# raahii/dcvgan

Hardware: AMD Instinct MI355X
Metric: videos/sec per G+D step, 16x64x64 RGB+depth (higher is better)
Workload: dtype f32

## Files before the change

### dcvgan_amd/csrc/conv_mfma.hip

```cpp
#include "dcv_common.h"

#include <algorithm>
#include <cstdlib>
#include <map>
#include <mutex>
#include <string>
#include <type_traits>
#include <vector>

namespace dcv {

thread_local char g_err[512] = {0};
std::atomic<uint64_t> g_launches{0};
thread_local char g_last_kernel[160] = {0};
#define DCV_NOTE_KERNEL(...) snprintf(g_last_kernel, sizeof(g_last_kernel), __VA_ARGS__)

typedef float f32x16 __attribute__((ext_vector_type(16)));
typedef __bf16 bf16x8 __attribute__((ext_vector_type(8)));

std::atomic<int> g_precision{0};
struct BnView {
    const float* bx; const float* gamma; const float* beta; const float* mean; const float* invstd;
    int64_t bx_sn;
    int32_t bx_sc, bx_sh, cbn, act;
// ... 1409 lines not shown
    uint32_t plane, gb;
    xcd_plane_map(blockIdx.x, gpp, gridDim.x, plane, gb);
    const uint32_t n = plane / (uint32_t)a.OD, od = plane - n * (uint32_t)a.OD;
    int32_t kb4[KS];
    uint32_t padmask = 0, b0mask = 0, b2mask = 0, r0mask = 0, r1mask = 0, r2mask = 0;
#pragma unroll
    for (int m = 0; m < KS; ++m) {
        const int k = 2 * m + lhi;
        const bool live = k < K;
        const int kk = live ? k : 0;
        const int rc = kk / 9, t = kk - rc * 9, ra = t / 3, b = t - ra * 3;
        kb4[m] = rc * a.s_stepA + 4 * (ra * a.x_sh + b);
        padmask |= live ? 0u : 1u << m;
        b0mask |= (live && b == 0) ? 1u << m : 0u;
        b2mask |= (live && b == 2) ? 1u << m : 0u;
        r0mask |= (live && ra == 0) ? 1u << m : 0u;
        r1mask |= (live && ra == 1) ? 1u << m : 0u;
        r2mask |= (live && ra == 2) ? 1u << m : 0u;
    }
    const __amdgpu_buffer_rsrc_t xrs = __builtin_amdgcn_make_buffer_rsrc(
        const_cast<float*>(a.x + (int64_t)n * a.x_sn + (int64_t)((int)od * a.td.mul + a.td.base + a.td.delta[0]) * a.x_sd), 0, 0x80000000u, 0x00020000);
    const __amdgpu_buffer_rsrc_t yrs = __builtin_amdgcn_make_buffer_rsrc(a.y + a.y_off + (int64_t)n * a.y_sn + (int64_t)od * a.y_sd, 0, 0x80000000u, 0x00020000);
    const __amdgpu_buffer_rsrc_t bxrs = __builtin_amdgcn_make_buffer_rsrc(const_cast<float*>(h.bx + (int64_t)n * h.bx_sn), 0, 0x80000000u, 0x00020000);
    const __amdgpu_buffer_rsrc_t bdrs = __builtin_amdgcn_make_buffer_rsrc((MODE == 2 ? h.bdx : a.y) + (MODE == 2 ? (int64_t)n * h.bdx_sn : 0), 0, 0x80000000u, 0x00020000);
    const int ysh = (int)a.y_sh, ysw = (int)a.y_sw;
    const uint32_t ysc4 = (uint32_t)a.y_sc * 4u, bxsc4 = (uint32_t)h.bx_sc * 4u, bdsc4 = (uint32_t)h.bdx_sc * 4u;
    const float slope = h.slope;

    auto load_b = [&](int oh, int x0, float (&bv)[KS]) {
        const int ih0 = oh + a.p_ihmin;
        const int col = x0 + l31;
        uint32_t bad = padmask | (col == 0 ? b0mask : 0u) | (col == a.tw.size - 1 ? b2mask : 0u);
        if ((unsigned)ih0 >= (unsigned)a.th.size) bad |= r0mask;
        if ((unsigned)(ih0 + 1) >= (unsigned)a.th.size) bad |= r1mask;
        if ((unsigned)(ih0 + 2) >= (unsigned)a.th.size) bad |= r2mask;
        const int base4 = 4 * (ih0 * a.x_sh + col - 1);
#pragma unroll
        for (int m = 0; m < KS; ++m) {
            const uint32_t vo = ((bad >> m) & 1u) ? 0x80000000u : (uint32_t)(base4 + kb4[m]);
            bv[m] = __builtin_bit_cast(float, __builtin_amdgcn_raw_buffer_load_b32(xrs, vo, 0, 0));
        }
    };

    const int ntile = groups * 2;
    __syncthreads();
    const int ohw = (int)gb * groups * 4 + wave * groups;
    const int mt_end = MODE == 2 ? MB : MT;
#pragma unroll 1
    for (int mt = 0; mt < mt_end; ++mt) {
        const bool bn = mt < MB;
        float af[KS];
#pragma unroll
        for (int m = 0; m < KS; ++m) af[m] = wl[2 * m + lhi][mt * 32 + l31];
        float s1[16], s2[16];
#pragma unroll
        for (int r = 0; r < 16; ++r) { s1[r] = 0.f; s2[r] = 0.f; }
        float bcur[KS], bnxt[KS];
        load_b(ohw, 0, bcur);
#pragma unroll 1
        for (int tt = 0; tt < ntile; ++tt) {
            const int oh = ohw + (tt >> 1), x0 = (tt & 1) * 32;
            float xt[16];
            if (bn) {
                const uint32_t xv = (uint32_t)(4 * (oh * h.bx_sh + (x0 + l31) * h.bx_sw)) + (uint32_t)(4 * lhi) * bxsc4;
#pragma unroll
                for (int r = 0; r < 16; ++r)
                    xt[r] = __builtin_bit_cast(float, __builtin_amdgcn_raw_buffer_load_b32(bxrs, xv, (uint32_t)(mt * 32 + (r & 3) + 8 * (r >> 2)) * bxsc4, 0));
            }
            if (tt + 1 < ntile) load_b(ohw + ((tt + 1) >> 1), ((tt + 1) & 1) * 32, bnxt);
            f32x16 acc;
#pragma unroll
            for (int r = 0; r < 16; ++r) acc[r] = 0.f;
#pragma unroll
            for (int m = 0; m < KS; ++m) acc = __builtin_amdgcn_mfma_f32_32x32x2f32(af[m], bcur[m], acc, 0, 0, 0);
            if (bn) {
                const uint32_t dv = (uint32_t)(4 * (oh * h.bdx_sh + (x0 + l31) * h.bdx_sw)) + (uint32_t)(4 * lhi) * bdsc4;
#pragma unroll
                for (int r = 0; r < 16; ++r) {
                    const int ch = mt * 32 + (r & 3) + 8 * (r >> 2) + 4 * lhi;
                    const f32x4 k4 = c4[ch];
                    const float z = xt[r] * k4[0] + k4[1];
                    const float dz = acc[r] * (z > 0.f ? 1.f : slope);
                    const float xm = xt[r] - k4[2];
                    if (MODE == 1) {
                        s1[r] += dz;
                        s2[r] += dz * xm;
                    } else {
                        const f32x2 k2 = c2[ch];
                        const float o = k4[0] * dz + k2[0] + k2[1] * xm;
                        __builtin_amdgcn_raw_buffer_store_b32(__builtin_bit_cast(int, o), bdrs, dv, (uint32_t)(mt * 32 + (r & 3) + 8 * (r >> 2)) * bdsc4, 2);
                    }
                }
            } else {
                const uint32_t yv = (uint32_t)(4 * (oh * ysh + (x0 + l31) * ysw)) + (uint32_t)(4 * lhi) * ysc4;
#pragma unroll
                for (int r = 0; r < 16; ++r) {
                    const float v = acc[r];
                    __builtin_amdgcn_raw_buffer_store_b32(__builtin_bit_cast(int, v), yrs, yv, (uint32_t)(mt * 32 + (r & 3) + 8 * (r >> 2)) * ysc4, 2);
                }
            }
#pragma unroll
            for (int m = 0; m < KS; ++m) bcur[m] = bnxt[m];
        }
        if (MODE == 1 && bn) {
#pragma unroll
            for (int r = 0; r < 16; ++r) {
                const float t1 = half_wave_sum(s1[r]), t2 = half_wave_sum(s2[r]);
                if (l31 == 31) {
                    const int ch = mt * 32 + (r & 3) + 8 * (r >> 2) + 4 * lhi;
                    red[wave][ch][0] = t1;
                    red[wave][ch][1] = t2;
                }
            }
        }
    }
    if (MODE == 1) {
        __syncthreads();
        if (tid < 2 * cbn) {
            const int ch = tid >> 1, w = tid & 1;
            h.partial[((int64_t)blockIdx.x * cbn + ch) * 2 + w] = ((red[0][ch][w] + red[1][ch][w]) + red[2][ch][w]) + red[3][ch][w];
        }
    }
}

__global__ __launch_bounds__(256) void head_bn_finalize_kernel(const float* __restrict__ partial, int nwg, int cbn, double count, const float* __restrict__ gamma,
                                                               const float* __restrict__ invstd, float* __restrict__ dgamma, float* __restrict__ dbeta, float* __restrict__ cst) {
    __shared__ double red[2][256];
    const int c = blockIdx.x, tid = threadIdx.x;
    double a0 = 0.0, a1 = 0.0;
    for (int w = tid; w < nwg; w += 256) {
        a0 += (double)partial[((int64_t)w * cbn + c) * 2];
        a1 += (double)partial[((int64_t)w * cbn + c) * 2 + 1];
    }
    red[0][tid] = a0; red[1][tid] = a1;
    __syncthreads();
    for (int st = 128; st > 0; st >>= 1) {
        if (tid < st) { red[0][tid] += red[0][tid + st]; red[1][tid] += red[1][tid + st]; }
        __syncthreads();
    }
    if (tid == 0) {
        const double is = (double)invstd[c], sc = (double)gamma[c] * is;
        const double S1 = red[0][0], S2 = red[1][0];
        dbeta[c] = (float)S1;
        dgamma[c] = (float)(S2 * is);
        cst[2 * c] = (float)(-sc * S1 / count);
        cst[2 * c + 1] = (float)(-sc * is * is * S2 / count);
    }
}

struct QuadArgs {
    const float* s;
    float* y;
    const float* w;
    int32_t N, RC, OC, SD, SH, OD, pad0, pad1;
    int64_t s_sn, s_sc, s_sd, s_sh;
    int64_t y_sn, y_sc, y_sd, y_sh;
    int64_t w_o, w_r;
    int32_t act, accumulate;
    float slope, pad2;
};

template <int NOC, int ND>
__global__ __launch_bounds__(256) void thin_quad_kernel(const QuadArgs a) {
    __shared__ float red[3][8 * NOC][64];
    const int tid = threadIdx.x, lane = tid & 63;
    const int wave = __builtin_amdgcn_readfirstlane(tid >> 6);
    const int col = lane & 31, hw = lane >> 5;
    const uint32_t qb = (uint32_t)a.SH >> 2;
    const uint32_t plane = blockIdx.x / qb;
    const int r0 = (int)(blockIdx.x - plane * qb) * 4 + 2 * hw;
    const uint32_t n = plane / (uint32_t)a.OD, od = plane - n * (uint32_t)a.OD;
    int roff[4];
#pragma unroll
    for (int i = 0; i < 4; ++i) {
        const int rr = r0 - 1 + i;
        roff[i] = (unsigned)rr < (unsigned)a.SH ? rr * (int)a.s_sh + col : -1;
    }
    float acc[2][2][2][NOC];
#pragma unroll
    for (int q = 0; q < 2; ++q)
#pragma unroll
        for (int h = 0; h < 2; ++h)
#pragma unroll
            for (int b = 0; b < 2; ++b)
#pragma unroll
                for (int c = 0; c < NOC; ++c) acc[q][h][b][c] = 0.f;
    const float* __restrict__ sn = a.s + (int64_t)n * a.s_sn;
#pragma unroll(ND == 1 ? 4 : 1)
    for (int rc = wave; rc < a.RC; rc += 4) {
        float ctr[ND][4];
#pragma unroll
        for (int kd = 0; kd < ND; ++kd) {
            const int sd = (int)od - kd;
            const bool in = (unsigned)sd < (unsigned)a.SD;
            const float* __restrict__ pl = sn + (int64_t)rc * a.s_sc + (int64_t)(in ? sd : 0) * a.s_sd;
#pragma unroll
            for (int i = 0; i < 4; ++i) ctr[kd][i] = (in && roff[i] >= 0) ? pl[roff[i]] : 0.f;
        }
#pragma unroll
        for (int kd = 0; kd < ND; ++kd) {
            float g[4][3];
#pragma unroll
            for (int i = 0; i < 4; ++i) {
                const float v = ctr[kd][i];
                g[i][1] = v;
                float l = __builtin_bit_cast(float, __builtin_amdgcn_update_dpp(0, __builtin_bit_cast(int, v), 0x138, 0xf, 0xf, true));
                float r = __builtin_bit_cast(float, __builtin_amdgcn_update_dpp(0, __builtin_bit_cast(int, v), 0x130, 0xf, 0xf, true));
                g[i][0] = col == 0 ? 0.f : l;
                g[i][2] = col == 31 ? 0.f : r;
            }
#pragma unroll
            for (int c = 0; c < NOC; ++c) {
                if (c >= a.OC) continue;
                typedef float f32x4 __attribute__((ext_vector_type(4)));
                const f32x4* __restrict__ wq = reinterpret_cast<const f32x4*>(a.w + (int64_t)c * a.w_o + (int64_t)rc * a.w_r + kd * 16);
                const f32x4 w0 = wq[0], w1 = wq[1], w2 = wq[2], w3 = wq[3];
#pragma unroll
                for (int q = 0; q < 2; ++q) {
                    const float (&top)[3] = g[q], (&mid)[3] = g[q + 1], (&bot)[3] = g[q + 2];
                    acc[q][0][0][c] += mid[1] * w1[1] + mid[0] * w1[3] + top[1] * w3[1] + top[0] * w3[3];
                    acc[q][0][1][c] += mid[2] * w1[0] + mid[1] * w1[2] + top[2] * w3[0] + top[1] * w3[2];
                    acc[q][1][0][c] += bot[1] * w0[1] + bot[0] * w0[3] + mid[1] * w2[1] + mid[0] * w2[3];
                    acc[q][1][1][c] += bot[2] * w0[0] + bot[1] * w0[2] + mid[2] * w2[0] + mid[1] * w2[2];
                }
            }
        }
    }
    if (wave > 0) {
#pragma unroll
        for (int q = 0; q < 2; ++q)
#pragma unroll
            for (int h = 0; h < 2; ++h)
#pragma unroll
                for (int b = 0; b < 2; ++b)
#pragma unroll
                    for (int c = 0; c < NOC; ++c) red[wave - 1][((q * 2 + h) * 2 + b) * NOC + c][lane] = acc[q][h][b][c];
    }
    __syncthreads();
    if (wave != 0) return;
    const int OC = a.OC, act = a.act, accumulate = a.accumulate;
    const float slope = a.slope;
    float* __restrict__ yb = a.y + (int64_t)n * a.y_sn + (int64_t)od * a.y_sd + 2 * col;
#pragma unroll
    for (int q = 0; q < 2; ++q)
#pragma unroll
        for (int h = 0; h < 2; ++h)
#pragma unroll
            for (int c = 0; c < NOC; ++c) {
                if (c >= OC) continue;
                float v[2];
#pragma unroll
                for (int b = 0; b < 2; ++b) {
                    const int e = ((q * 2 + h) * 2 + b) * NOC + c;
                    v[b] = acc[q][h][b][c] + ((red[0][e][lane] + red[1][e][lane]) + red[2][e][lane]);
                }
                float* dst = yb + (int64_t)(2 * (r0 + q) + h) * a.y_sh + (int64_t)c * a.y_sc;
                if (accumulate) { v[0] += dst[0]; v[1] += dst[1]; }
                dst[0] = apply_act(v[0], act, slope);
                dst[1] = apply_act(v[1], act, slope);
            }
}

template <int T>
static bool launch_thin_struct(const GatherArgs& a, int OC, int RC, int rc_per_split, dim3 grid, hipStream_t s) {
    switch (OC) {
        case 1: hipLaunchKernelGGL((thin_struct_kernel<T, 1>), grid, dim3(256), 0, s, a, RC, rc_per_split); return true;
        case 2: hipLaunchKernelGGL((thin_struct_kernel<T, 2>), grid, dim3(256), 0, s, a, RC, rc_per_split); return true;
        case 3: hipLaunchKernelGGL((thin_struct_kernel<T, 3>), grid, dim3(256), 0, s, a, RC, rc_per_split); return true;
        case 4: hipLaunchKernelGGL((thin_struct_kernel<T, 4>), grid, dim3(256), 0, s, a, RC, rc_per_split); return true;
    }
    return false;
}

struct PackArgs {
    const KEntry* ktab[4];
    float* wp[4];
    int32_t K16[4];
    int32_t fmt[4];
};
__global__ void pack_weights_kernel(const float* __restrict__ w, const PackArgs pa, int OC, int OCp, int64_t ws_o) {
    const int c = blockIdx.y;
    const int64_t i = (int64_t)blockIdx.x * blockDim.x + threadIdx.x;
    if (i >= (int64_t)pa.K16[c] * OCp) return;
    const int k = (int)(i / OCp), oc = (int)(i % OCp);
    const KEntry e = pa.ktab[c][k];
    float v = 0.f;
    if (oc < OC && !(e.tapsel >> 31)) v = w[(int64_t)oc * ws_o + e.w_off];
    if (pa.fmt[c] == 2) {
        if (X6_PHASE(k >> 4)) v = -v;
        __bf16* o = reinterpret_cast<__bf16*>(pa.wp[c]);
        const __bf16 hi = (__bf16)v;
        const float r = v - (float)hi;
        const __bf16 mid = (__bf16)r;
        const __bf16 lo = (__bf16)(r - (float)mid);
        const int64_t base = (((int64_t)(k >> 4) * 6 + ((k >> 3) & 1)) * OCp + oc) * 8 + (k & 7);
        o[base] = hi; o[base + (int64_t)2 * OCp * 8] = mid; o[base + (int64_t)4 * OCp * 8] = lo;
    } else if (pa.fmt[c]) reinterpret_cast<__bf16*>(pa.wp[c])[((int64_t)(k >> 3) * OCp + oc) * 8 + (k & 7)] = (__bf16)v;
    else pa.wp[c][i] = v;
}

struct WgradArgs {
    const float* dptr;
    const float* gptr;
    float* slab;
    const KEntry* jtab;
    int32_t M, DC, J, DCp, Jp, chunk, pad0, pad1;
    FastDiv div_sp, div_hw, div_w;
    DimTaps td, th, tw;
    int64_t d_sn, g_sn;
    int32_t d_sc4, d_sd, d_sh, d_sw;
    int32_t g_sd, g_sh, g_sw, pad2;
    int32_t g_sc4, g_sd4, log2nd, pad3;
    int32_t hw_off4[16];
    uint32_t hw_sel[16];
};

template <int TD, int TJ, int WD, int WJ, bool REG16>
__global__ __launch_bounds__(256, (TD * TJ >= 4 ? (REG16 ? 3 : 2) : 3)) void wgrad_gemm_kernel(const WgradArgs a) {
    constexpr int BD = 32 * TD * WD;
    constexpr int BJ = 32 * TJ * WJ;
    constexpr int DPT = BD / 8, JPT = BJ / 8;
    static_assert(WD * WJ == 4, "4 waves");
    __shared__ float Ds[32][BD + 1];
    __shared__ float Gs[32][BJ + 1];

    const int tid = threadIdx.x;
    const int lane = tid & 63;
    const int wave = __builtin_amdgcn_readfirstlane(tid >> 6);
    const int wd = wave / WJ, wj = wave % WJ;
    const int tiles_d = a.DCp / BD;
    const int d_t = blockIdx.x % tiles_d, j_t = blockIdx.x / tiles_d;
    const int d0 = d_t * BD, j0 = j_t * BJ;
    const int ml = tid & 31, sub = tid >> 5;

    const int m_begin = blockIdx.y * a.chunk;
    const int m_end = min(a.M, m_begin + a.chunk);
    const int nit = (m_end > m_begin) ? (m_end - m_begin + 31) / 32 : 0;

    const uint32_t nb = fdiv((uint32_t)(nit > 0 ? m_begin : 0), a.div_sp);
    const __amdgpu_buffer_rsrc_t drs = __builtin_amdgcn_make_buffer_rsrc(const_cast<float*>(a.dptr + (int64_t)nb * a.d_sn), 0, 0x80000000u, 0x00020000);
    const __amdgpu_buffer_rsrc_t grs = __builtin_amdgcn_make_buffer_rsrc(const_cast<float*>(a.gptr + (int64_t)nb * a.g_sn), 0, 0x40000000u, 0x00020000);

    int32_t goff4[REG16 ? 1 : JPT];
    uint32_t gsel[REG16 ? 1 : JPT];
    int32_t gso[REG16 ? JPT / 2 : 1];
    uint32_t jmask = 0;
    int32_t tapA = 0, tapB = 0;
    uint32_t selA = 0, selB = 0;
    if constexpr (REG16) {
        const int subu = sub & 7;
        tapA = a.hw_off4[subu]; tapB = a.hw_off4[subu + 8];
        selA = a.hw_sel[subu]; selB = a.hw_sel[subu + 8];
#pragma unroll
        for (int q = 0; q < JPT / 2; ++q) {
            const int cd = j0 / 16 + q;
            gso[q] = (cd >> a.log2nd) * a.g_sc4 + (cd & ((1 << a.log2nd) - 1)) * a.g_sd4;
        }
#pragma unroll
        for (int i = 0; i < JPT; ++i)
            if (j0 + sub + 8 * i < a.J) jmask |= 1u << i;
    } else {
#pragma unroll
        for (int i = 0; i < JPT; ++i) {
            const int j = j0 + sub + 8 * i;
            if (j < a.J) {
                const KEntry e = a.jtab[j];
                goff4[i] = e.x_off * 4;
                gsel[i] = e.tapsel;
            } else {
                goff4[i] = 0;
                gsel[i] = 1u << 31;
            }
        }
    }
    const int dcb4 = (d0 + sub) * a.d_sc4;
    const int dstep4 = 8 * a.d_sc4;
    uint32_t dcmask = 0;
#pragma unroll
    for (int i = 0; i < DPT; ++i)
        if (d0 + sub + 8 * i < a.DC) dcmask |= 1u << i;

    f32x16 acc[TD][TJ];
#pragma unroll
    for (int i = 0; i < TD; ++i)
#pragma unroll
        for (int j = 0; j < TJ; ++j)
#pragma unroll
            for (int r = 0; r < 16; ++r) acc[i][j][r] = 0.f;

    float dv[DPT], gv[JPT];

    auto load_tile = [&](int it) {
        const int m = m_begin + it * 32 + ml;
        const bool mok = m < m_end;
        const int mm = mok ? m : m_begin;
        const uint32_t n = fdiv((uint32_t)mm, a.div_sp);
        uint32_t r = (uint32_t)mm - n * a.div_sp.div;
        const uint32_t pd = fdiv(r, a.div_hw);
        r -= pd * a.div_hw.div;
        const uint32_t ph = fdiv(r, a.div_w);
        const uint32_t pw = r - ph * a.div_w.div;
        const int dbase4 = 4 * ((int)((int64_t)(n - nb) * a.d_sn) + (int)pd * a.d_sd + (int)ph * a.d_sh + (int)pw * a.d_sw) + dcb4;
        const uint32_t dm = mok ? dcmask : 0u;
#pragma unroll
        for (int i = 0; i < DPT; ++i) {
            const uint32_t vo = ((dm >> i) & 1u) ? (uint32_t)(dbase4 + i * dstep4) : 0x80000000u;
            dv[i] = __builtin_bit_cast(float, __builtin_amdgcn_raw_buffer_load_b32(drs, vo, 0, 0));
        }
        const uint32_t vmask = mok ? (dim_mask(a.td, (int)pd, 0) | dim_mask(a.th, (int)ph, 8) | dim_mask(a.tw, (int)pw, 16)) : 0u;
        const int gbase4 = 4 * ((int)((int64_t)(n - nb) * a.g_sn) + ((int)pd * a.td.mul + a.td.base) * a.g_sd +
                                ((int)ph * a.th.mul + a.th.base) * a.g_sh + ((int)pw * a.tw.mul + a.tw.base) * a.g_sw);
        if constexpr (REG16) {
            const uint32_t voA = ((vmask & selA) == selA) ? (uint32_t)(gbase4 + tapA) : 0x80000000u;
// ... 2097 lines not shown
        else
            hipLaunchKernelGGL(wgrad_reduce_kernel, dim3((unsigned)((32 * J + 63) / 64)), dim3(256), 0, stream, slab, R, P.nslab, 32, J, 32, J, acc);
        break;
    }
    case WK::Tiled: {
        const int GC = op.gd.c, *k = op.k;
        const dcv_dims5& gd = op.gd;
        char kb[512];
        const int nn = snprintf(kb, sizeof(kb), "%s|w|%d|%d,%d,%d|%lld|%lld|%lld|%lld", op.tag, GC, k[0], k[1], k[2], (long long)gd.sc, (long long)gd.sd, (long long)gd.sh, (long long)gd.sw);
        DevTable tab;
        const int rc = get_table(device_prefix() + std::string(kb, nn), [&] {
            std::vector<KEntry> host;
            for (int gc = 0; gc < GC; ++gc)
                for (int ud = 0; ud < k[0]; ++ud)
                    for (int uh = 0; uh < k[1]; ++uh)
                        for (int uw = 0; uw < k[2]; ++uw)
                            host.push_back(KEntry{(int32_t)((int64_t)gc * gd.sc + (int64_t)ud * gd.sd + (int64_t)uh * gd.sh + (int64_t)uw * gd.sw),
                                                  (1u << ud) | (1u << (8 + uh)) | (1u << (16 + uw)), 0, 0});
            return host;
        }, &tab);
        if (rc != DCV_OK) return rc;
        WgradArgs a = P.g;
        a.dptr = D; a.gptr = G; a.slab = slab; a.jtab = tab.dev;
        const WgradTile tc = P.tc;
        const int gx = (int)P.grid.x, S2 = P.nslab;
        if (P.dma >= 0) DCV_NOTE_KERNEL("wgrad_dma_kernel<%d, %d, %s> (%d x %d tile, %d slabs%s)", tc.bd == 128 ? 2 : 1, P.dma, P.d16 ? "true" : "false", tc.bd, tc.bj, S2,
                                        P.dma == 2 ? ", f32x6: fp32 on the bf16 pipe" : P.dma ? ", bf16 products" : "");
        else DCV_NOTE_KERNEL("wgrad_gemm_kernel (%d x %d tile, %d slabs)", tc.bd, tc.bj, S2);
        if (P.dma == 2) {
            if (tc.bd == 128) hipLaunchKernelGGL((wgrad_dma_kernel<2, 2>), P.grid, dim3(256), 0, stream, a);
            else hipLaunchKernelGGL((wgrad_dma_kernel<1, 2>), P.grid, dim3(256), 0, stream, a);
        } else if (P.dma == 1) {
            if (tc.bd == 128) hipLaunchKernelGGL((wgrad_dma_kernel<2, 1>), P.grid, dim3(256), 0, stream, a);
            else hipLaunchKernelGGL((wgrad_dma_kernel<1, 1>), P.grid, dim3(256), 0, stream, a);
        } else if (P.dma == 0 && P.d16) {
            hipLaunchKernelGGL((wgrad_dma_kernel<1, 0, true>), P.grid, dim3(256), 0, stream, a);
        } else if (P.dma == 0) {
            if (tc.bd == 128) hipLaunchKernelGGL((wgrad_dma_kernel<2, 0>), P.grid, dim3(256), 0, stream, a);
            else hipLaunchKernelGGL((wgrad_dma_kernel<1, 0>), P.grid, dim3(256), 0, stream, a);
        }
        else if (tc.bd == 128 && tc.bj == 32) launch_wgrad<1, 1, 4, 1>(a, gx, S2, stream);
        else if (tc.bd == 128 && tc.bj == 128) launch_wgrad<2, 2, 2, 2>(a, gx, S2, stream);
        else if (tc.bd == 128 && tc.bj == 64) launch_wgrad<2, 1, 2, 2>(a, gx, S2, stream);
        else if (tc.bd == 64 && tc.bj == 256) launch_wgrad<2, 2, 1, 4>(a, gx, S2, stream);
        else if (tc.bd == 64 && tc.bj == 128) launch_wgrad<2, 1, 1, 4>(a, gx, S2, stream);
        else if (tc.bd == 32 && tc.bj == 256) launch_wgrad<1, 2, 1, 4>(a, gx, S2, stream);
        else launch_wgrad<1, 1, 1, 4>(a, gx, S2, stream);
        DCV_LAUNCH_CHECK();
        const int J = a.J, Jp = a.Jp, DCp = a.DCp;
        const int64_t tot = (int64_t)DC * J;
        if (J % 4 == 0 && Jp % 4 == 0 && (reinterpret_cast<uintptr_t>(R) & 15) == 0)
            hipLaunchKernelGGL(wgrad_reduce4_kernel, dim3((unsigned)((tot / 4 + 63) / 64)), dim3(256), 0, stream, slab, R, S2, DC, J, DCp, Jp, acc);
        else
            hipLaunchKernelGGL(wgrad_reduce_kernel, dim3((unsigned)((tot + 63) / 64)), dim3(256), 0, stream, slab, R, S2, DC, J, DCp, Jp, acc);
        break;
    }
    }
    DCV_LAUNCH_CHECK();
    return DCV_OK;
}
}

using namespace dcv;

extern "C" {

int dcv_debug_kernel_info(char* buf, size_t n) {
    struct Item { const char* name; const void* fn; };
    const Item items[] = {
        {"gather<2,2,2,2,S>", (const void*)gather_gemm_kernel<2, 2, 2, 2, true>}, {"gather<2,2,1,4,S>", (const void*)gather_gemm_kernel<2, 2, 1, 4, true>},
        {"gather<1,2,1,4,S>", (const void*)gather_gemm_kernel<1, 2, 1, 4, true>}, {"gather<2,2,2,2,T>", (const void*)gather_gemm_kernel<2, 2, 2, 2, false>},
        {"gather_dma<2,2,2,2>", (const void*)gather_gemm_dma_kernel<2, 2, 2, 2, false, false>}, {"gather_dma<2,2,1,4>", (const void*)gather_gemm_dma_kernel<2, 2, 1, 4, false, false>},
        {"gather_dma<1,2,1,4>", (const void*)gather_gemm_dma_kernel<1, 2, 1, 4, false, false>}, {"gather_dma_patch<2,2,2,2>", (const void*)gather_gemm_dma_kernel<2, 2, 2, 2, false, true>},
        {"thin_gather", (const void*)thin_gather_kernel},
        {"wgrad_dma", (const void*)wgrad_dma_kernel<2>}, {"wgrad_dma64", (const void*)wgrad_dma_kernel<1>}, {"wgrad<2,2,2,2,R>", (const void*)wgrad_gemm_kernel<2, 2, 2, 2, true>}, {"wgrad<2,2,1,4,R>", (const void*)wgrad_gemm_kernel<2, 2, 1, 4, true>},
        {"wgrad<2,2,2,2>", (const void*)wgrad_gemm_kernel<2, 2, 2, 2, false>}, {"wgrad<2,1,2,2>", (const void*)wgrad_gemm_kernel<2, 1, 2, 2, false>},
        {"wgrad<2,2,1,4>", (const void*)wgrad_gemm_kernel<2, 2, 1, 4, false>}, {"wgrad<2,1,1,4>", (const void*)wgrad_gemm_kernel<2, 1, 1, 4, false>},
        {"wgrad<1,2,1,4>", (const void*)wgrad_gemm_kernel<1, 2, 1, 4, false>}, {"wgrad<1,1,1,4>", (const void*)wgrad_gemm_kernel<1, 1, 1, 4, false>},
    };
    size_t off = 0;
    for (const Item& it : items) {
        int blocks = -1;
        hipFuncAttributes at;
        memset(&at, 0, sizeof(at));
        hipError_t e1 = hipOccupancyMaxActiveBlocksPerMultiprocessor(&blocks, it.fn, 256, 0);
        hipError_t e2 = hipFuncGetAttributes(&at, it.fn);
        int w = snprintf(buf + off, off < n ? n - off : 0, "%s: blocks/CU=%d regs=%d lds=%zu scratch=%zu (%s)\n", it.name, blocks, at.numRegs,
                         (size_t)at.sharedSizeBytes, (size_t)at.localSizeBytes, (e1 == hipSuccess && e2 == hipSuccess) ? "ok" : "query failed");
        if (w < 0) break;
        off += (size_t)w;
        if (off >= n) break;
    }
    return (int)off;
}

#ifdef DCV_STAMP
int dcv_debug_read_stamps(unsigned long long* host, int nblocks) {
    return (int)hipMemcpyFromSymbol(host, HIP_SYMBOL(g_stamp), sizeof(unsigned long long) * 24 * (size_t)nblocks, 0, hipMemcpyDeviceToHost);
}
#endif

const char* dcv_last_error(void) { return g_err; }
const char* dcv_debug_last_kernel(void) { return g_last_kernel; }
int dcv_set_precision(int mode) {
    if (mode < 0 || mode > 2) return fail(DCV_EINVAL, "set_precision: 0 = fp32, 1 = bf16 MFMA products, 2 = fp32 emulated on the bf16 matrix pipe (3 x bf16 split, 6 products)");
    g_precision.store(mode);
    return DCV_OK;
}
int dcv_get_precision(void) { return g_precision.load(); }
int dcv_version(void) { return 4; }
void dcv_abi_struct_sizes(size_t out[3]) {
    if (!out) return;
    out[0] = sizeof(dcv_dims5); out[1] = sizeof(dcv_conv_geom); out[2] = sizeof(dcv_wpack);
}
int dcv_conv_effective_precision(const dcv_conv_geom* g) {
    if (g && g->mfma >= 1 && g->mfma <= 3) return g->mfma;
    return g_precision.load() + 1;
}
uint64_t dcv_launch_count(void) { return g_launches.load(); }


static bool latent_form(const dcv_conv_geom* g, const dcv_dims5* x, const dcv_dims5* y, dcv_conv_geom* g2, dcv_dims5* y2) {
    if (!g || !x || !y || !g->transposed) return false;
    const int T = g->kd * g->kh * g->kw;
    if (T <= 1 || x->d != 1 || x->h != 1 || x->w != 1 || g->sd != 1 || g->sh != 1 || g->sw != 1 || g->pd || g->ph || g->pw) return false;
    if (y->d != g->kd || y->h != g->kh || y->w != g->kw || y->c != g->cout || (int64_t)g->cout * T >= (1ll << 30)) return false;
    const int64_t sw = 1, sh = y->w, sd = (int64_t)y->h * y->w, sc = (int64_t)y->d * y->h * y->w;
    if ((y->w > 1 && y->sw != sw) || (y->h > 1 && y->sh != sh) || (y->d > 1 && y->sd != sd) || (y->c > 1 && y->sc != sc)) return false;
    *g2 = *g;
    g2->kd = g2->kh = g2->kw = 1;
    g2->cout = g->cout * T;
    *y2 = *y;
    y2->c = g->cout * T; y2->d = y2->h = y2->w = 1;
    y2->sc = 1; y2->sd = y2->sh = y2->sw = 0;
    return true;
}



static bool plan_thin_quad(const dcv_dims5& sd_, const dcv_dims5& dd, const int k[3], const int s[3], const int p[3], int act, float slope, int accumulate, QuadArgs* a) {
    if (toggles().no_quad) return false;
    const int OC = dd.c, RC = sd_.c;
    if (OC > 4 || k[1] != 4 || k[2] != 4 || s[1] != 2 || s[2] != 2 || p[1] != 1 || p[2] != 1 || s[0] != 1 || p[0] != 0 || (k[0] != 1 && k[0] != 4)) return false;
    if (sd_.w != 32 || dd.w != 64 || dd.h != 2 * sd_.h || sd_.h % 4 != 0 || sd_.sw != 1 || dd.sw != 1) return false;
    if (dd.d != sd_.d + k[0] - 1) return false;
    if ((int64_t)dd.n * dd.d * (sd_.h / 4) >= (1ll << 31) || sd_.sh * (int64_t)sd_.h >= (1ll << 30)) return false;
    memset(a, 0, sizeof(*a));
    a->N = dd.n; a->RC = RC; a->OC = OC; a->SD = sd_.d; a->SH = sd_.h; a->OD = dd.d;
    a->s_sn = sd_.sn; a->s_sc = sd_.sc; a->s_sd = sd_.sd; a->s_sh = sd_.sh;
    a->y_sn = dd.sn; a->y_sc = dd.sc; a->y_sd = dd.sd; a->y_sh = dd.sh;
    const int T = k[0] * 16;
    a->w_o = T; a->w_r = (int64_t)OC * T;
    a->act = act; a->slope = slope; a->accumulate = accumulate;
    return true;
}
static int run_thin_quad(QuadArgs a, const float* src, float* dst, const float* w, int kd, hipStream_t stream) {
    a.s = src; a.y = dst; a.w = w;
    const dim3 grid((unsigned)((int64_t)a.N * a.OD * (a.SH / 4)));
#define DCV_QUAD(NOC_)                                                                                          \
    {                                                                                                           \
        if (kd == 1) hipLaunchKernelGGL((thin_quad_kernel<NOC_, 1>), grid, dim3(256), 0, stream, a);            \
        else hipLaunchKernelGGL((thin_quad_kernel<NOC_, 4>), grid, dim3(256), 0, stream, a);                    \
    }
    switch (a.OC) {
        case 1: DCV_QUAD(1) break;
        case 2: DCV_QUAD(2) break;
        case 3: DCV_QUAD(3) break;
        default: DCV_QUAD(4) break;
    }
#undef DCV_QUAD
    DCV_NOTE_KERNEL("thin_quad_kernel<%d, %d>", a.OC, kd);
    DCV_LAUNCH_CHECK();
    return DCV_OK;
}

struct ConvCall {
    int which = 0;
    const dcv_conv_geom* g = nullptr;
    const dcv_dims5 *xd = nullptr, *yd = nullptr;
    const float* src = nullptr; const float* w = nullptr; float* dst = nullptr;
    int act = DCV_ACT_NONE, accumulate = 0; float slope = 0.f;
    bool stats = false; float* stat = nullptr; size_t stat_bytes = 0;
    const dcv_wpack* pack = nullptr;
    const float* gate = nullptr; float gate_slope = 0.f;
};
enum class ConvPath { Gather, HeadFwd, HeadDgrad, Quad };
struct ConvPlan {
    ConvPath path = ConvPath::Gather;
    dcv_conv_geom g{}; dcv_dims5 xd{}, yd{};
    GatherOp op;
    GatherPlan gp;
    QuadArgs quad;
    size_t ws_need = 0;
};

static int plan_conv(const ConvCall& c, const CallOpts& o, ConvPlan* P, bool sizes = false) {
    if (c.which != 0 && c.which != 1) return fail(DCV_EINVAL, "conv: bad dispatch");
    if (!c.g || !c.xd || !c.yd) return fail(DCV_EINVAL, "conv: null descriptor");
    const bool latent = !c.gate && latent_form(c.g, c.xd, c.yd, &P->g, &P->yd);
    if (!latent) { P->g = *c.g; P->yd = *c.yd; }
    P->xd = *c.xd;
    const dcv_conv_geom& g = P->g;
    const dcv_dims5 &xd = P->xd, &yd = P->yd;
    const int rc0 = check_geom(&g, &xd, &yd, "conv");
    if (rc0 != DCV_OK) return rc0;
    const int which = c.which;
    const int k[3] = {g.kd, g.kh, g.kw}, s[3] = {g.sd, g.sh, g.sw}, p[3] = {g.pd, g.ph, g.pw};
    const int xi[3] = {xd.d, xd.h, xd.w}, yo[3] = {yd.d, yd.h, yd.w};
    const int T = k[0] * k[1] * k[2];
    const dcv_dims5& src = which == 0 ? xd : yd;
    const dcv_dims5& dst = which == 0 ? yd : xd;
    GatherOp& op = P->op;
    op = GatherOp();
    op.x = c.src; op.xd = src; op.y = c.dst; op.yd = dst; op.w = c.w;
    op.RC = src.c; op.OC = dst.c; op.KH = k[1]; op.KW = k[2];
    const bool direct = (which == 0 && !g.transposed) || (which == 1 && g.transposed);
    if (direct) {
        op.classes = direct_classes(k, s, p, which == 0 ? yo : xi, which == 0 ? xi : yo);
        op.ws_o = (int64_t)op.RC * T; op.ws_r = T;
    } else {
        op.classes = scatter_classes(k, s, p, which == 0 ? yo : xi, which == 0 ? xi : yo);
        op.ws_o = T; op.ws_r = (int64_t)op.OC * T;
    }
    op.act = c.act; op.slope = c.slope; op.accumulate = c.accumulate;
    op.stats = c.stats && !latent;
    op.stat = c.stat; op.stat_bytes = c.stat_bytes; op.pack = c.pack; op.gate = c.gate; op.gate_slope = c.gate_slope;
    op.tag = which == 0 ? (g.transposed ? "convT_fwd" : "conv_fwd") : (g.transposed ? "convT_bwd_data" : "conv_bwd_data");
    const bool head = !op.stats && !c.gate && head_shape_ok(k, s, p, g.transposed != 0, xd, yd, o.precision);
    P->path = ConvPath::Gather;
    P->ws_need = 0;
    if (head && which == 0 && k[0] == 4) {
        P->path = ConvPath::HeadFwd;
        P->ws_need = head_fwd_bytes(xd, k[0]);
    } else if (head && which == 1 && k[0] == 1) P->path = ConvPath::HeadDgrad;
    else if (!direct && !op.stats && !c.gate && plan_thin_quad(src, dst, k, s, p, c.act, c.slope, c.accumulate, &P->quad)) P->path = ConvPath::Quad;
    if (P->path != ConvPath::Gather && !sizes) return DCV_OK;
    const int rc = plan_gather(op, o, &P->gp);
    if (rc != DCV_OK) return rc;
    P->ws_need = std::max(P->ws_need, P->gp.ws_need);
    return DCV_OK;
}

static int run_conv(const ConvCall& c, const ConvPlan& P, const CallOpts& o, void* ws, size_t ws_bytes, void* stream, int* stat_parts = nullptr) {
    if (stat_parts) *stat_parts = 0;
    if (c.pack && c.pack->buf && c.pack->precision != o.precision + 1)
        return fail(DCV_EINVAL, "conv: dcv_wpack.precision is %d but this call runs at precision %d (1 fp32, 2 bf16 products, 3 fp32-on-bf16): %s",
                    c.pack->precision, o.precision + 1, c.pack->ready ? "a ready pack of another format would be read" : "stamp the buffer with dcv_conv_effective_precision(g)");
    if (!c.src || !c.w || !c.dst) return fail(DCV_EINVAL, "conv: null pointer");
    if (P.ws_need > ws_bytes) return fail(DCV_EWORKSPACE, "%s: workspace too small (%zu needed, %zu given)", P.op.tag, P.ws_need, ws_bytes);
    hipStream_t st = static_cast<hipStream_t>(stream);
    switch (P.path) {
    case ConvPath::HeadFwd: return run_head_fwd(c.src, P.xd, c.w, c.dst, P.yd, P.g.kd, c.act, c.slope, ws, st);
    case ConvPath::HeadDgrad: return run_head_dgrad(c.src, P.yd, c.w, c.dst, P.xd, P.g.kd, c.accumulate, st);
    case ConvPath::Quad: return run_thin_quad(P.quad, c.src, c.dst, c.w, P.g.kd, st);
    case ConvPath::Gather: break;
    }
    if (c.pack && c.pack->buf && P.gp.pack_need > c.pack->bytes)
        return fail(DCV_EWORKSPACE, "%s: packed-weight buffer too small (%zu needed, %zu given)", P.op.tag, P.gp.pack_need, c.pack->bytes);
    const int rc = run_gather(P.op, P.gp, o, c.pack, ws, st);
    if (rc == DCV_OK && stat_parts) *stat_parts = P.gp.stat_parts;
    return rc;
}

static int conv_call(const ConvCall& c, void* ws, size_t ws_bytes, void* stream) {
    CallOpts o; ConvPlan P;
    int rc = call_opts(c.g, &o, "conv");
    if (rc == DCV_OK) rc = plan_conv(c, o, &P);
    return rc == DCV_OK ? run_conv(c, P, o, ws, ws_bytes, stream) : rc;
}

static int plan_wgrad_call(const dcv_conv_geom* g, const float* x, const dcv_dims5* xd, const float* dy, const dcv_dims5* dyd, float* dw, const CallOpts& o,
                           WgradOp* op, WgradPlan* P) {
    dcv_conv_geom g2; dcv_dims5 y2;
    if (latent_form(g, xd, dyd, &g2, &y2)) { g = &g2; dyd = &y2; }
    const int rc = check_geom(g, xd, dyd, "conv_bwd_weight");
    if (rc != DCV_OK) return rc;
    if (o.bnview && !g->transposed) return fail(DCV_EUNSUPPORTED, "conv_bwd_weight: BatchNorm on load reads the dense operand: the input of a transposed convolution");
    const int k[3] = {g->kd, g->kh, g->kw}, s[3] = {g->sd, g->sh, g->sw}, p[3] = {g->pd, g->ph, g->pw};
    for (int d = 0; d < 3; ++d) { op->k[d] = k[d]; op->s[d] = s[d]; op->p[d] = p[d]; }
    if (!g->transposed) { op->D = dy; op->dd = *dyd; op->G = x; op->gd = *xd; op->tag = "conv_bwd_weight"; }
    else { op->D = x; op->dd = *xd; op->G = dy; op->gd = *dyd; op->tag = "convT_bwd_weight"; }
    op->R = dw;
    return plan_wgrad(*op, o, P);
}

static int wgrad_call(const dcv_conv_geom* g, const float* x, const dcv_dims5* xd, const float* dy, const dcv_dims5* dyd, float* dw,
                      void* ws, size_t ws_bytes, void* stream, const CallOpts& o) {
    WgradOp op; WgradPlan P;
    int rc = plan_wgrad_call(g, x, xd, dy, dyd, dw, o, &op, &P);
    if (rc != DCV_OK) return rc;
    if (!x || !dy || !dw || !ws) return fail(DCV_EINVAL, "conv_bwd_weight: null pointer");
    if (o.bnview && !P.bn)
        return fail(DCV_EUNSUPPORTED, "conv_backward_weight_bn: not the 3-channel 3x3 transposed head on 64-wide rows with 128 k input channels and a 16-byte aligned BatchNorm input");
    if (P.need > ws_bytes) return fail(DCV_EWORKSPACE, "%s: workspace too small (%zu needed, %zu given)", op.tag, P.need, ws_bytes);
    return run_wgrad(op, P, o, ws, static_cast<hipStream_t>(stream));
}

static int plan_sizes(const dcv_conv_geom* g, const dcv_dims5* x, const dcv_dims5* y, int which, bool stats, ConvPlan* P) {
    CallOpts o; ConvCall c;
    c.which = which; c.g = g; c.xd = x; c.yd = y; c.stats = stats;
    const int rc = call_opts(g, &o, "conv");
    return rc != DCV_OK ? rc : plan_conv(c, o, P, true);
}

size_t dcv_conv_workspace_bytes(const dcv_conv_geom* g, const dcv_dims5* x, const dcv_dims5* y, int which) {
    if (which != 2) { ConvPlan P; return plan_sizes(g, x, y, which, false, &P) == DCV_OK ? P.ws_need : 0; }
    CallOpts o; WgradOp op; WgradPlan P, t;
    if (call_opts(g, &o, "conv") != DCV_OK || plan_wgrad_call(g, nullptr, x, nullptr, y, nullptr, o, &op, &P) != DCV_OK) return 0;
    if ((P.kind == WK::ThinJ || P.kind == WK::Stem3d) && plan_tiled_wgrad(op, o, &t) == DCV_OK) return std::max(P.need, t.need);
    return P.need;
}

size_t dcv_conv_backward_data_bn_workspace_bytes(const dcv_dims5* dx, int cbn) {
    if (!dx || cbn < 1) return 0;
    return align_up((size_t)dx->n * dx->d * ((dx->h + 3) / 4) * cbn * 2 * sizeof(float), 256) + align_up((size_t)cbn * 2 * sizeof(float), 256) + 256;
}

int dcv_conv_backward_data_bn(const dcv_conv_geom* g, const float* dy, const dcv_dims5* dyd, const float* w, float* dx, const dcv_dims5* dxd, const dcv_wpack* pack,
                              void* ws, size_t ws_bytes, int cbn, const float* bn_x, const dcv_dims5* bn_xd, const float* gamma, const float* beta,
                              const float* save_mean, const float* save_invstd, int act, float slope, float* bn_dx, const dcv_dims5* bn_dxd, float* dgamma, float* dbeta,
                              void* ws2, size_t ws2_bytes, int* fused, void* stream) {
    if (!fused || !bn_x || !bn_xd || !gamma || !beta || !save_mean || !save_invstd || !bn_dx || !bn_dxd || !dgamma || !dbeta || !dxd || !ws2)
        return fail(DCV_EINVAL, "conv_backward_data_bn: null pointer");
    *fused = 0;
// ... 138 lines not shown
```

Baseline: 649.2.

## Add fp32 MFMA variant of thin quad transposed-conv kernel for channel reduction

Adds an MFMA-based path for the thin output-channel stride-2 4x4 transposed convolution. It computes per-tap partial products with 16x16x4 fp32 MFMA over 32-channel chunks using buffer loads, stages them in shared memory, and then combines the taps into output pixels. The existing VALU kernel is kept as a fallback when channels are not a multiple of 32 or OC is large. The aim is to move the channel reduction onto matrix cores, at the cost of extra LDS traffic, barriers and zero-initialisation per block.

Result: no change. 654.8 (median of 6 runs) (+0.9%).

```diff
diff --git a/dcvgan_amd/csrc/conv_mfma.hip b/dcvgan_amd/csrc/conv_mfma.hip
--- a/dcvgan_amd/csrc/conv_mfma.hip
+++ b/dcvgan_amd/csrc/conv_mfma.hip
@@ -1585,7 +1585,7 @@
     const float* s;
     float* y;
     const float* w;
-    int32_t N, RC, OC, SD, SH, OD, pad0, pad1;
+    int32_t N, RC, OC, SD, SH, OD, mfma, pad1;
     int64_t s_sn, s_sc, s_sd, s_sh;
     int64_t y_sn, y_sc, y_sd, y_sh;
     int64_t w_o, w_r;
@@ -1594,7 +1594,7 @@
 };
 
 template <int NOC, int ND>
-__global__ __launch_bounds__(256) void thin_quad_kernel(const QuadArgs a) {
+__device__ __forceinline__ void thin_quad_vector(const QuadArgs& a) {
     __shared__ float red[3][8 * NOC][64];
     const int tid = threadIdx.x, lane = tid & 63;
     const int wave = __builtin_amdgcn_readfirstlane(tid >> 6);
@@ -1692,6 +1692,104 @@
                 dst[0] = apply_act(v[0], act, slope);
                 dst[1] = apply_act(v[1], act, slope);
             }
+}
+
+template <int NOC, int ND>
+__device__ __forceinline__ void thin_quad_mfma(const QuadArgs& a) {
+    typedef float f32x4 __attribute__((ext_vector_type(4)));
+    constexpr int TP = 36;
+    __shared__ float T[NOC][6][16][TP];
+    const int tid = threadIdx.x, lane = tid & 63;
+    const int wave = __builtin_amdgcn_readfirstlane(tid >> 6);
+    const uint32_t qb = (uint32_t)a.SH >> 2;
+    const uint32_t plane = blockIdx.x / qb;
+    const int r0 = (int)(blockIdx.x - plane * qb) * 4;
+    const uint32_t n = plane / (uint32_t)a.OD, od = plane - n * (uint32_t)a.OD;
+    for (int i = tid; i < NOC * 6 * 16 * TP; i += 256) (&T[0][0][0][0])[i] = 0.f;
+    const int l15 = lane & 15, lq = lane >> 4;
+    const int i0 = wave >> 1, c0 = (wave & 1) * 16;
+    uint32_t boff[3];
+#pragma unroll
+    for (int j = 0; j < 3; ++j) {
+        const int rr = r0 - 1 + i0 + 2 * j;
+        boff[j] = (unsigned)rr < (unsigned)a.SH ? 4u * (uint32_t)(lq * (int)a.s_sc + rr * (int)a.s_sh + c0 + l15) : 0x80000000u;
+    }
+    const uint32_t ssc16 = 16u * (uint32_t)a.s_sc, wr16 = 16u * (uint32_t)a.w_r;
+    const int col = lane & 31, h = lane >> 5, q = wave;
+    const float* __restrict__ ta = &T[0][q + 1 + h][(1 - h) * 4][col];
+    const float* __restrict__ tb = &T[0][q + h][(3 - h) * 4][col];
+    float acc[2][NOC];
+#pragma unroll
+    for (int c = 0; c < NOC; ++c) acc[0][c] = acc[1][c] = 0.f;
+    const float* __restrict__ sn = a.s + (int64_t)n * a.s_sn;
+    const __amdgpu_buffer_rsrc_t wrs = __builtin_amdgcn_make_buffer_rsrc(const_cast<float*>(a.w), 0, 0x80000000u, 0x00020000);
+    const uint32_t woff = 4u * (uint32_t)(lq * (int)a.w_r + l15);
+#pragma unroll 1
+    for (int kd = 0; kd < ND; ++kd) {
+        const int sd = (int)od - kd;
+        if ((unsigned)sd >= (unsigned)a.SD) continue;
+        const __amdgpu_buffer_rsrc_t srs = __builtin_amdgcn_make_buffer_rsrc(const_cast<float*>(sn + (int64_t)sd * a.s_sd), 0, 0x80000000u, 0x00020000);
+        f32x4 t[NOC][3];
+#pragma unroll
+        for (int c = 0; c < NOC; ++c)
+#pragma unroll
+            for (int j = 0; j < 3; ++j) t[c][j] = f32x4{0.f, 0.f, 0.f, 0.f};
+#pragma unroll 1
+        for (int rc0 = 0; rc0 < a.RC; rc0 += 32) {
+            float bf[3][8];
+#pragma unroll
+            for (int j = 0; j < 3; ++j)
+#pragma unroll
+                for (int ks = 0; ks < 8; ++ks)
+                    bf[j][ks] = __builtin_bit_cast(float, __builtin_amdgcn_raw_buffer_load_b32(srs, boff[j], (uint32_t)(rc0 / 4 + ks) * ssc16, 0));
+#pragma unroll
+            for (int c = 0; c < NOC; ++c) {
+                float af[8];
+#pragma unroll
+                for (int ks = 0; ks < 8; ++ks)
+                    af[ks] = __builtin_bit_cast(float, __builtin_amdgcn_raw_buffer_load_b32(wrs, woff, (uint32_t)(rc0 / 4 + ks) * wr16 + 4u * (uint32_t)(c * (int)a.w_o + kd * 16), 0));
+#pragma unroll
+                for (int ks = 0; ks < 8; ++ks)
+#pragma unroll
+                    for (int j = 0; j < 3; ++j) t[c][j] = __builtin_amdgcn_mfma_f32_16x16x4f32(af[ks], bf[j][ks], t[c][j], 0, 0, 0);
+            }
+        }
+        __syncthreads();
+#pragma unroll
+        for (int c = 0; c < NOC; ++c)
+#pragma unroll
+            for (int j = 0; j < 3; ++j)
+#pragma unroll
+                for (int r = 0; r < 4; ++r) {
+                    const float v = t[c][j][r];
+                    T[c][i0 + 2 * j][4 * lq + r][1 + c0 + l15] = v;
+                }
+        __syncthreads();
+#pragma unroll
+        for (int c = 0; c < NOC; ++c) {
+            const float* __restrict__ pa = ta + c * (6 * 16 * TP);
+            const float* __restrict__ pb = tb + c * (6 * 16 * TP);
+            acc[0][c] += ((pa[1 * TP + 1] + pa[3 * TP]) + pb[1 * TP + 1]) + pb[3 * TP];
+            acc[1][c] += ((pa[2] + pa[2 * TP + 1]) + pb[2]) + pb[2 * TP + 1];
+        }
+    }
+    const int act = a.act, accumulate = a.accumulate;
+    const float slope = a.slope;
+    float* __restrict__ yb = a.y + (int64_t)n * a.y_sn + (int64_t)od * a.y_sd + (int64_t)(2 * (r0 + q) + h) * a.y_sh + 2 * col;
+#pragma unroll
+    for (int c = 0; c < NOC; ++c) {
+        float* dst = yb + (int64_t)c * a.y_sc;
+        float v0 = acc[0][c], v1 = acc[1][c];
+        if (accumulate) { v0 += dst[0]; v1 += dst[1]; }
+        dst[0] = apply_act(v0, act, slope);
+        dst[1] = apply_act(v1, act, slope);
+    }
+}
+
+template <int NOC, int ND, bool MFMA>
+__global__ __launch_bounds__(256) void thin_quad_kernel(const QuadArgs a) {
+    if constexpr (MFMA) thin_quad_mfma<NOC, ND>(a);
+    else thin_quad_vector<NOC, ND>(a);
 }
 
 template <int T>
@@ -4095,24 +4193,35 @@
     const int T = k[0] * 16;
     a->w_o = T; a->w_r = (int64_t)OC * T;
     a->act = act; a->slope = slope; a->accumulate = accumulate;
+    a->mfma = RC % 32 == 0 && OC <= 3 && !(OC == 3 && k[0] == 1) && sd_.sc >= 0 && sd_.sd >= 0 && sd_.sh >= 0 && (int64_t)RC * OC * T < (1ll << 28) &&
+              (int64_t)sd_.d * sd_.sd + (int64_t)RC * sd_.sc + sd_.sh * (int64_t)sd_.h < (1ll << 28);
     return true;
 }
 static int run_thin_quad(QuadArgs a, const float* src, float* dst, const float* w, int kd, hipStream_t stream) {
     a.s = src; a.y = dst; a.w = w;
     const dim3 grid((unsigned)((int64_t)a.N * a.OD * (a.SH / 4)));
-#define DCV_QUAD(NOC_)                                                                                          \
+#define DCV_QUAD(NOC_)                                                                                            \
     {                                                                                                           \
-        if (kd == 1) hipLaunchKernelGGL((thin_quad_kernel<NOC_, 1>), grid, dim3(256), 0, stream, a);            \
-        else hipLaunchKernelGGL((thin_quad_kernel<NOC_, 4>), grid, dim3(256), 0, stream, a);                    \
-    }
-    switch (a.OC) {
+        if (kd == 1) hipLaunchKernelGGL((thin_quad_kernel<NOC_, 1, false>), grid, dim3(256), 0, stream, a);     \
+        else hipLaunchKernelGGL((thin_quad_kernel<NOC_, 4, false>), grid, dim3(256), 0, stream, a);             \
+    }
+    if (a.mfma && kd == 1) switch (a.OC) {
+        case 1: hipLaunchKernelGGL((thin_quad_kernel<1, 1, true>), grid, dim3(256), 0, stream, a); break;
+        default: hipLaunchKernelGGL((thin_quad_kernel<2, 1, true>), grid, dim3(256), 0, stream, a); break;
+    }
+    else if (a.mfma) switch (a.OC) {
+        case 1: hipLaunchKernelGGL((thin_quad_kernel<1, 4, true>), grid, dim3(256), 0, stream, a); break;
+        case 2: hipLaunchKernelGGL((thin_quad_kernel<2, 4, true>), grid, dim3(256), 0, stream, a); break;
+        default: hipLaunchKernelGGL((thin_quad_kernel<3, 4, true>), grid, dim3(256), 0, stream, a); break;
+    }
+    else switch (a.OC) {
         case 1: DCV_QUAD(1) break;
         case 2: DCV_QUAD(2) break;
         case 3: DCV_QUAD(3) break;
         default: DCV_QUAD(4) break;
     }
 #undef DCV_QUAD
-    DCV_NOTE_KERNEL("thin_quad_kernel<%d, %d>", a.OC, kd);
+    DCV_NOTE_KERNEL("thin_quad_kernel<%d, %d>%s", a.OC, kd, a.mfma ? ", per-tap fp32 MFMA 16x16x4 over the gathered channels, 4-row bands" : "");
     DCV_LAUNCH_CHECK();
     return DCV_OK;
 }
```
